# taraak/pita

Hardware: AMD Instinct MI355X
Metric: walker-steps/sec (batch x T) LJ13 @ 65k walkers/GPU (higher is better)
Workload: dtype f32

## Files before the change

### pita_amd/csrc/egnn_common.h

```cpp
#pragma once
#include <cstdlib>

#include "common.h"

namespace pita {

typedef float f32x16 __attribute__((ext_vector_type(16)));
typedef float f32x4 __attribute__((ext_vector_type(4)));

constexpr int EH = 32;
constexpr int PBS = 36;
constexpr int MAT_F = 1024;
enum { M_WA = 0, M_WB, M_W2, M_WC1, M_WN1A, M_WN1B, M_WN2,
       M_WAT, M_WBT, M_W2T, M_WC1T, M_WN1AT, M_WN1BT, M_WN2T, M_COUNT };
enum { V_WRE = 0 , V_B1 = 2, V_B2, V_WATT, V_BC1, V_WC2, V_BN1,
       V_BN2, V_WRF , V_WEF , V_COUNT };
constexpr int VEC_EMB_F = 96;
constexpr int VEC_LAYER_F = V_COUNT * EH + 4;


__device__ __forceinline__ void wave_lds_fence() {
  asm volatile("s_waitcnt lgkmcnt(0)" ::: "memory");
}

// ... 10 lines not shown
  const f32x4* p = reinterpret_cast<const f32x4*>(v);
  f32x4 a = p[0], b = p[1], c = p[2], d = p[3];
  f32x16 r;
  r[0] = a.x; r[1] = a.y; r[2] = a.z; r[3] = a.w;
  r[4] = b.x; r[5] = b.y; r[6] = b.z; r[7] = b.w;
  r[8] = c.x; r[9] = c.y; r[10] = c.z; r[11] = c.w;
  r[12] = d.x; r[13] = d.y; r[14] = d.z; r[15] = d.w;
  return r;
}

typedef short bf16x8 __attribute__((ext_vector_type(8)));
typedef unsigned int u32x4 __attribute__((ext_vector_type(4)));
constexpr int MAT_W = 1536;

template <int PREC>
struct WFrag;

template <>
struct WFrag<0> {
  float wf[16];
  __device__ __forceinline__ void load(const float* __restrict__ m32, const unsigned* __restrict__, int mat, int lane) {
    const f32x4* p = reinterpret_cast<const f32x4*>(m32 + (size_t)mat * MAT_F) + lane;
#pragma unroll
    for (int q = 0; q < 4; ++q) {
      f32x4 v = p[q * 64];
      wf[4 * q + 0] = v.x; wf[4 * q + 1] = v.y; wf[4 * q + 2] = v.z; wf[4 * q + 3] = v.w;
    }
  }
  __device__ __forceinline__ f32x16 mul(const f32x16& in, f32x16 acc) const {
#pragma unroll
    for (int r = 0; r < 16; ++r) acc = __builtin_amdgcn_mfma_f32_32x32x2f32(wf[r], in[r], acc, 0, 0, 0);
    return acc;
  }
};

__device__ __forceinline__ bf16x8 as_bf16x8(u32x4 v) { return __builtin_bit_cast(bf16x8, v); }

template <>
struct WFrag<1> {
  u32x4 w[3][2];
  __device__ __forceinline__ void load(const float* __restrict__, const unsigned* __restrict__ m16, int mat, int lane) {
    const u32x4* p = reinterpret_cast<const u32x4*>(m16 + (size_t)mat * MAT_W) + lane;
#pragma unroll
    for (int pc = 0; pc < 3; ++pc)
#pragma unroll
      for (int st = 0; st < 2; ++st) w[pc][st] = p[(pc * 2 + st) * 64];
  }
  static __device__ __forceinline__ void split(const f32x16& in, u32x4 (&x)[3][2]) {
#pragma unroll
    for (int st = 0; st < 2; ++st)
#pragma unroll
      for (int q = 0; q < 4; ++q) {
        typedef float f32x2_t __attribute__((ext_vector_type(2)));
        const unsigned a = __float_as_uint(in[8 * st + 2 * q]), b = __float_as_uint(in[8 * st + 2 * q + 1]);
        const unsigned a1 = a & 0xFFFF0000u, b1 = b & 0xFFFF0000u;
        const f32x2_t r1 = f32x2_t{__uint_as_float(a), __uint_as_float(b)} - f32x2_t{__uint_as_float(a1), __uint_as_float(b1)};
        const unsigned ar = __float_as_uint(r1.x), br = __float_as_uint(r1.y);
        const unsigned a2 = ar & 0xFFFF0000u, b2 = br & 0xFFFF0000u;
        const f32x2_t r2 = r1 - f32x2_t{__uint_as_float(a2), __uint_as_float(b2)};
        const unsigned a3 = __float_as_uint(r2.x), b3 = __float_as_uint(r2.y);
        x[0][st][q] = __builtin_amdgcn_perm(b1, a1, 0x07060302u);
        x[1][st][q] = __builtin_amdgcn_perm(b2, a2, 0x07060302u);
        x[2][st][q] = __builtin_amdgcn_perm(b3, a3, 0x07060302u);
      }
  }
  __device__ __forceinline__ f32x16 mul_split(const u32x4 (&x)[3][2], f32x16 acc) const {
#pragma unroll
    for (int st = 0; st < 2; ++st) {
      acc = __builtin_amdgcn_mfma_f32_32x32x16_bf16(as_bf16x8(w[2][st]), as_bf16x8(x[0][st]), acc, 0, 0, 0);
      acc = __builtin_amdgcn_mfma_f32_32x32x16_bf16(as_bf16x8(w[0][st]), as_bf16x8(x[2][st]), acc, 0, 0, 0);
      acc = __builtin_amdgcn_mfma_f32_32x32x16_bf16(as_bf16x8(w[1][st]), as_bf16x8(x[1][st]), acc, 0, 0, 0);
      acc = __builtin_amdgcn_mfma_f32_32x32x16_bf16(as_bf16x8(w[1][st]), as_bf16x8(x[0][st]), acc, 0, 0, 0);
      acc = __builtin_amdgcn_mfma_f32_32x32x16_bf16(as_bf16x8(w[0][st]), as_bf16x8(x[1][st]), acc, 0, 0, 0);
      acc = __builtin_amdgcn_mfma_f32_32x32x16_bf16(as_bf16x8(w[0][st]), as_bf16x8(x[0][st]), acc, 0, 0, 0);
    }
    return acc;
  }
  __device__ __forceinline__ f32x16 mul(const f32x16& in, f32x16 acc) const {
    u32x4 x[3][2];
    split(in, x);
    return mul_split(x, acc);
  }
};

constexpr float F16_SX = 1.0f, F16_SW = 16.0f;
constexpr bool F16_NODE_LAYERS = true;
constexpr float F16_UNSCALE = 1.0f / (F16_SX * F16_SW);
constexpr float DIV_ST = 32.0f;
constexpr float DIV_SV = 2048.0f;
constexpr int VEC_DIV_F = 4 * EH;
constexpr int MAT_WH = 1024;
typedef _Float16 f16x8 __attribute__((ext_vector_type(8)));
typedef _Float16 f16x2 __attribute__((ext_vector_type(2)));
__device__ __forceinline__ f16x8 as_f16x8(u32x4 v) { return __builtin_bit_cast(f16x8, v); }
__device__ __forceinline__ float f16_rem_lo(unsigned pk, float x) {
  float r;
  asm("v_fma_mix_f32 %0, %1, -1.0, %2 op_sel:[0,0,0] op_sel_hi:[1,0,0]" : "=v"(r) : "v"(pk), "v"(x));
  return r;
}
__device__ __forceinline__ float f16_rem_hi(unsigned pk, float x) {
  float r;
  asm("v_fma_mix_f32 %0, %1, -1.0, %2 op_sel:[1,0,0] op_sel_hi:[1,0,0]" : "=v"(r) : "v"(pk), "v"(x));
  return r;
}

template <>
struct WFrag<2> {
  u32x4 w[2][2];
  __device__ __forceinline__ void load(const float* __restrict__, const unsigned* __restrict__ m16, int mat, int lane) {
    const u32x4* p = reinterpret_cast<const u32x4*>(m16 + (size_t)mat * MAT_WH) + lane;
#pragma unroll
    for (int pc = 0; pc < 2; ++pc)
#pragma unroll
      for (int st = 0; st < 2; ++st) w[pc][st] = p[(pc * 2 + st) * 64];
  }
  static __device__ __forceinline__ void split(const f32x16& in, u32x4 (&x)[2][2]) {
    typedef float f32x2_t __attribute__((ext_vector_type(2)));
#pragma unroll
    for (int st = 0; st < 2; ++st)
#pragma unroll
      for (int q = 0; q < 4; ++q) {
        const float a = in[8 * st + 2 * q], b = in[8 * st + 2 * q + 1];
        const unsigned p1 = __builtin_bit_cast(unsigned, __builtin_convertvector(f32x2_t{a, b}, f16x2));
        const float ra = f16_rem_lo(p1, a), rb = f16_rem_hi(p1, b);
        x[0][st][q] = p1;
        x[1][st][q] = __builtin_bit_cast(unsigned, __builtin_convertvector(f32x2_t{ra, rb}, f16x2));
      }
  }
  __device__ __forceinline__ f32x16 mul_split(const u32x4 (&x)[2][2], f32x16 acc) const {
#pragma unroll
    for (int st = 0; st < 2; ++st) {
      acc = __builtin_amdgcn_mfma_f32_32x32x16_f16(as_f16x8(w[1][st]), as_f16x8(x[0][st]), acc, 0, 0, 0);
      acc = __builtin_amdgcn_mfma_f32_32x32x16_f16(as_f16x8(w[0][st]), as_f16x8(x[1][st]), acc, 0, 0, 0);
      acc = __builtin_amdgcn_mfma_f32_32x32x16_f16(as_f16x8(w[0][st]), as_f16x8(x[0][st]), acc, 0, 0, 0);
    }
    return acc;
  }
  __device__ __forceinline__ f32x16 mul(const f32x16& in, f32x16 acc) const {
    u32x4 x[2][2];
    split(in, x);
    return mul_split(x, acc);
  }
};

typedef float f32x2 __attribute__((ext_vector_type(2)));
constexpr float SILU_PRESCALE = -1.44269504088896341f;
__device__ __forceinline__ f32x2 silu2(f32x2 v) {
  f32x2 e;
  e.x = __builtin_amdgcn_exp2f(v.x);
  e.y = __builtin_amdgcn_exp2f(v.y);
  const f32x2 d = e + 1.0f;
  f32x2 r;
  r.x = __builtin_amdgcn_rcpf(d.x);
  r.y = __builtin_amdgcn_rcpf(d.y);
  return v * r;
}
__device__ __forceinline__ void silu16(f32x16& m) {
  f32x2 e[8];
#pragma unroll
  for (int q = 0; q < 8; ++q) {
    e[q].x = __builtin_amdgcn_exp2f(m[2 * q]);
    e[q].y = __builtin_amdgcn_exp2f(m[2 * q + 1]);
  }
#pragma unroll
  for (int q = 0; q < 8; ++q) e[q] = e[q] + 1.0f;
#pragma unroll
// ... 28 lines not shown
  const f32x2 c = {1.0f / F16_SX, 1.0f / F16_SX};
#pragma unroll
  for (int q0 = 0; q0 < 8; q0 += Q) {
    f32x2 v[Q], e[Q];
#pragma unroll
    for (int q = 0; q < Q; ++q) {
      v[q] = f32x2{m[2 * (q0 + q)], m[2 * (q0 + q) + 1]};
      if (UNSCALE) v[q] = v[q] * F16_UNSCALE;
    }
#pragma unroll
    for (int q = 0; q < Q; ++q) {
      e[q].x = __builtin_amdgcn_exp2f(v[q].x);
      e[q].y = __builtin_amdgcn_exp2f(v[q].y);
    }
#pragma unroll
    for (int q = 0; q < Q; ++q) e[q] = __builtin_elementwise_fma(e[q], c, c);
#pragma unroll
    for (int q = 0; q < Q; ++q) {
      e[q].x = __builtin_amdgcn_rcpf(e[q].x);
      e[q].y = __builtin_amdgcn_rcpf(e[q].y);
    }
#pragma unroll
    for (int q = 0; q < Q; ++q) {
      const f32x2 y = v[q] * e[q];
      m[2 * (q0 + q)] = y.x;
      m[2 * (q0 + q) + 1] = y.y;
    }
  }
}
__device__ __forceinline__ void silu16_out(f32x16& m) { silu16_staged<false>(m); }
__device__ __forceinline__ void silu16_acc(f32x16& m) { silu16_staged<true>(m); }

__device__ __forceinline__ float dot16(const f32x16& w, const f32x16& m) {
  f32x2 acc = {0.f, 0.f};
#pragma unroll
  for (int q = 0; q < 8; ++q)
    acc = __builtin_elementwise_fma(f32x2{w[2 * q], w[2 * q + 1]}, f32x2{m[2 * q], m[2 * q + 1]}, acc);
  return acc.x + acc.y;
}

__device__ __forceinline__ float xhalf_sum(float v) {
  const unsigned u = __float_as_uint(v);
  const auto r = __builtin_amdgcn_permlane32_swap(u, u, false, false);
  return __uint_as_float(r[0]) + __uint_as_float(r[1]);
}

__device__ __forceinline__ void frag_to_agpr(WFrag<2>& f) {
#pragma unroll
  for (int pc = 0; pc < 2; ++pc)
#pragma unroll
    for (int st = 0; st < 2; ++st) asm volatile("" : "+a"(f.w[pc][st]));
}
__device__ __forceinline__ void frag_to_agpr(WFrag<1>& f) {
#pragma unroll
  for (int pc = 0; pc < 3; ++pc)
#pragma unroll
    for (int st = 0; st < 2; ++st) asm volatile("" : "+a"(f.w[pc][st]));
}

__device__ __forceinline__ float tanh_select(float v) {
  const float a = fabsf(v);
  const float v2 = v * v;
  float p = 62.0f / 2835.0f;
  p = fmaf(p, v2, -17.0f / 315.0f);
  p = fmaf(p, v2, 2.0f / 15.0f);
  p = fmaf(p, v2, -1.0f / 3.0f);
  p = fmaf(p, v2, 1.0f);
  float small = v * p;
  const float e = __builtin_amdgcn_exp2f(2.88539008177792681f * a);
  float big = copysignf(1.0f - 2.0f * __builtin_amdgcn_rcpf(1.0f + e), v);
  asm volatile("" : "+v"(small), "+v"(big));
  return a < 0.25f ? small : big;
}

}

struct pita_egnn {
  pita_egnn_config cfg;
  unsigned* d_mats16 = nullptr;
  unsigned* d_mats16h = nullptr;
  float* d_mats = nullptr;
  float* d_vecs = nullptr;
  float* d_vecs_h = nullptr;
  float* d_vecs_div = nullptr;
  int* d_vjp_mark = nullptr;
  size_t vjp_mark_bytes = 0;
  const void* shape = nullptr;
  const void* shape_small = nullptr;
  int n_cu = 256;
  int device = -1;
  float* d_ws = nullptr;
  size_t ws_bytes = 0;
  float* d_divcache = nullptr;
  size_t divcache_bytes = 0;
  int* d_mark = nullptr;
  size_t mark_bytes = 0;
  int div_seq = 0;
  float* d_probe_q = nullptr;
  size_t probe_q_bytes = 0;
  void* d_bk = nullptr;
  size_t bk_bytes = 0;
};
```

### pita_amd/csrc/egnn_kernel.hip

```cpp
#include "egnn_common.h"

namespace pita {

struct EgnnParams {
  const unsigned* mats16;
  const unsigned* mats16h;
  const float* mats;
  const float* vecs;
  int n_layers, in_nf, attention, tanh_on, feature_layout;
  float coord_scale;
  int mode;
  long long B;
  const float* x_in;
  const float* t;
  const float* beta;
  float* out;
  float* x;
  const float* step_tab;
  int n_steps;
  const float* noise;
  unsigned long long seed, walker_offset;
  long long step0;
  int remove_mean;
  float* drift_out;
  double* stats_out;
  int repair;
  const float* x_backup;
  int* bad_from;
};

#ifndef PITA_EGNN_RECOMPUTE_COLS
#define PITA_EGNN_RECOMPUTE_COLS 1
#endif

template <int N, int DIM, int G, int WAVES>
struct EgnnCfg {
  static constexpr int NCOL = G * N;
  static constexpr int NT = (NCOL + 31) / 32;
  static constexpr int NCOLP = NT * 32;
  static constexpr int PB_F = NCOLP * PBS;
  static constexpr int POS_F = NCOLP * DIM;
  static constexpr int WAVE_F = PB_F + 4 * POS_F;
  static __host__ __device__ constexpr int vec_f(int L) { return ((VEC_EMB_F + L * VEC_LAYER_F) + 3) & ~3; }
  static __host__ __device__ constexpr size_t lds_bytes(int L) {
    return sizeof(float) * (size_t)(vec_f(L) + WAVES * WAVE_F);
  }
};

template <int N, int DIM, int G, int WAVES, int PREC, bool SAMPLER, int OCC = 2>
__global__ void __launch_bounds__(WAVES * 64, OCC) egnn_kernel(EgnnParams p) {
  const int mode = SAMPLER ? 3 : p.mode;
  using C = EgnnCfg<N, DIM, G, WAVES>;
  constexpr int NT = C::NT;
  extern __shared__ __attribute__((aligned(16))) float lds[];

  const int L = p.n_layers;
  const int vec_f = C::vec_f(L);
  for (int i = threadIdx.x; i < VEC_EMB_F + L * VEC_LAYER_F; i += WAVES * 64) lds[i] = p.vecs[i];
  __syncthreads();

  const int wave = threadIdx.x >> 6;
  const int lane = threadIdx.x & 63;
  const int cl = lane & 31;
  const int hh = lane >> 5;
  float* PB = lds + vec_f + wave * C::WAVE_F;
  float* posbuf0 = PB + C::PB_F;
  float* posbuf1 = posbuf0 + C::POS_F;
  float* pos0 = posbuf1 + C::POS_F;
  float* xbuf = pos0 + C::POS_F;
  const float* vemb = lds;

  const long long total_waves = (long long)gridDim.x * WAVES;
  const long long quota = (p.B + total_waves - 1) / total_waves;
  const long long wbeg = ((long long)blockIdx.x * WAVES + wave) * quota;
  const long long wend = (wbeg + quota < p.B) ? wbeg + quota : p.B;
  for (long long walker0 = wbeg; walker0 < wend; walker0 += G) {
    const int nwalk = (int)((wend - walker0) < G ? (wend - walker0) : G);
    const int ncol = nwalk * N;
    const int ntile = (ncol + 31) >> 5;
    int col[NT], nodei[NT];
    bool valid[NT];
    long long wid[NT];
    float xcur[NT][DIM];
#pragma unroll
    for (int T = 0; T < NT; ++T) {
      col[T] = T * 32 + cl;
      int w = col[T] / N;
      nodei[T] = col[T] - w * N;
      wid[T] = walker0 + w;
      valid[T] = (col[T] < ncol);
      if (!valid[T]) wid[T] = p.B - 1;
      const float* src = (mode == 3 ? p.x : p.x_in);
#pragma unroll
      for (int k = 0; k < DIM; ++k) xcur[T][k] = valid[T] ? src[(walker0 * N + col[T]) * DIM + k] : 0.0f;
    }
    int bad_from[NT];
#pragma unroll
    for (int T = 0; T < NT; ++T) bad_from[T] = 0x7fffffff;
    bool mine[NT];
#pragma unroll
    for (int T = 0; T < NT; ++T) mine[T] = valid[T];
    if (PREC != 2 && p.repair) {
      bool bad = false;
      float* flag = PB;
#pragma unroll
      for (int T = 0; T < NT; ++T) {
        bool b = false;
#pragma unroll
        for (int k = 0; k < DIM; ++k) {
          const float v = (mode == 3) ? xcur[T][k] : (valid[T] ? p.out[(walker0 * N + col[T]) * DIM + k] : 0.0f);
          b = b || !__builtin_isfinite(v);
        }
        if (hh == 0) flag[col[T]] = b ? 1.0f : 0.0f;
        bad = bad || b;
      }
      if (!__any(bad)) continue;
      wave_lds_fence();
#pragma unroll
      for (int T = 0; T < NT; ++T) {
        const int cb = (col[T] < ncol) ? col[T] - nodei[T] : 0;
        float any = 0.f;
        for (int q = 0; q < N; ++q) any += flag[cb + q];
        mine[T] = valid[T] && any != 0.f;
      }
      wave_lds_fence();
      if (mode == 3) {
#pragma unroll
        for (int T = 0; T < NT; ++T) {
#pragma unroll
          for (int k = 0; k < DIM; ++k)
            xcur[T][k] = valid[T] ? p.x_backup[(walker0 * N + col[T]) * DIM + k] : 0.0f;
          if (p.stats_out && p.bad_from && valid[T]) bad_from[T] = p.bad_from[walker0 * N + col[T]];
        }
      }
    }

// ... 38 lines not shown
          c_s[T] = u_cs; c_in[T] = u_cin; c_out[T] = u_cout;
          tfeat[T] = u_cn; hval[T] = u_h; bfeat[T] = u_b;
        }
        g2 = uni(PITA_ST_G2); gamma = uni(PITA_ST_GAMMA); dt = uni(PITA_ST_DT);
        noise_scale = uni(PITA_ST_NOISE_SCALE); sqrt_dt = uni(PITA_ST_SQRT_DT);
      } else {
#pragma unroll
        for (int T = 0; T < NT; ++T) {
          float tv = p.t[wid[T]];
          bfeat[T] = p.beta ? p.beta[wid[T]] : 0.0f;
          if (mode == 0) {
            c_s[T] = 0.f; c_in[T] = 1.f; c_out[T] = 1.f; tfeat[T] = tv; hval[T] = 1.f;
          } else {
            hval[T] = tv;
            c_s[T] = 1.0f / (1.0f + tv);
            c_in[T] = 1.0f / sqrtf(1.0f + tv);
            c_out[T] = sqrtf(tv) * c_in[T];
            tfeat[T] = 0.125f * logf(tv);
          }
        }
      }

      f32x16 hfeat[NT];
#pragma unroll
      for (int T = 0; T < NT; ++T) {
#pragma unroll
        for (int k = 0; k < DIM; ++k) {
          const float xc = xbuf[col[T] * DIM + k];
          const float ps = (mode == 0) ? xc : c_in[T] * xc;
          if (hh == 0) {
            pos0[col[T] * DIM + k] = ps;
            posbuf0[col[T] * DIM + k] = ps;
          }
        }
        float a0, a1;
        if (p.in_nf == 1) {
          a0 = tfeat[T]; a1 = 0.f;
        } else if (p.feature_layout == 0) {
          a0 = (2 * nodei[T] < N) ? tfeat[T] : bfeat[T];
          a1 = (2 * nodei[T] + 1 < N) ? tfeat[T] : bfeat[T];
        } else {
          a0 = tfeat[T]; a1 = bfeat[T];
        }
        f32x16 w0 = lds_vec16(vemb + hh * 16), w1 = lds_vec16(vemb + 32 + hh * 16), eb = lds_vec16(vemb + 64 + hh * 16);
#pragma unroll
        for (int r = 0; r < 16; ++r) hfeat[T][r] = fmaf(w0[r], a0, fmaf(w1[r], a1, eb[r]));
      }
      wave_lds_fence();

      float* poscur = posbuf0;
      float* posnext = posbuf1;
      for (int l = 0; l < L; ++l) {
        const float* mats = p.mats + (size_t)l * M_COUNT * MAT_F;
        const unsigned* mats16 = p.mats16 + (size_t)l * M_COUNT * MAT_W;
        const unsigned* mats16h = p.mats16h + (size_t)l * M_COUNT * MAT_WH;
        constexpr int NPREC = (PREC == 2 && !F16_NODE_LAYERS) ? 1 : PREC;
        constexpr bool NODE16 = (PREC == 2 && F16_NODE_LAYERS);
        const unsigned* matsn = NODE16 ? mats16h : mats16;
        const float* vl = lds + VEC_EMB_F + l * VEC_LAYER_F + hh * 16;
        const bool last = (l == L - 1);
        const float aggw = last ? 0.0f : (PREC == 2 ? 1.0f / F16_SX : 1.0f);
        {
          WFrag<NPREC> wb;
          wb.load(mats, matsn, M_WB, lane);
#pragma unroll
          for (int T = 0; T < NT; ++T) {
            if (T >= ntile) continue;
            f32x16 z = {0};
            f32x16 pb = wb.mul(hfeat[T], z);
            if (NODE16) pb *= F16_UNSCALE;
            f32x4* dst = reinterpret_cast<f32x4*>(PB + col[T] * PBS + hh * 16);
            dst[0] = f32x4{pb[0], pb[1], pb[2], pb[3]};
            dst[1] = f32x4{pb[4], pb[5], pb[6], pb[7]};
            dst[2] = f32x4{pb[8], pb[9], pb[10], pb[11]};
            dst[3] = f32x4{pb[12], pb[13], pb[14], pb[15]};
          }
        }
        wave_lds_fence();

        WFrag<PREC> w2f, wc1f;
        w2f.load(mats, PREC == 2 ? mats16h : mats16, M_W2, lane);
        wc1f.load(mats, PREC == 2 ? mats16h : mats16, M_WC1, lane);
        const float a_re = lds[VEC_EMB_F + l * VEC_LAYER_F + V_WRE * EH + lane];
        const float b_att = lds[VEC_EMB_F + l * VEC_LAYER_F + V_COUNT * EH];

#pragma unroll
        for (int T = 0; T < NT; ++T) {
          if (T >= ntile) continue;
          f32x16 Ai;
          {
            WFrag<NPREC> wa;
            wa.load(mats, matsn, M_WA, lane);
            Ai = wa.mul(hfeat[T], lds_vec16(vl + V_B1 * EH));
            if (NODE16) Ai *= F16_UNSCALE;
          }
          f32x16 agg = {0};
          float xacc[DIM], pown[DIM], p0own[DIM];
#pragma unroll
          for (int k = 0; k < DIM; ++k) {
            xacc[k] = 0.f;
            pown[k] = poscur[col[T] * DIM + k];
            p0own[k] = pos0[col[T] * DIM + k];
          }
          const int cbase = col[T] - nodei[T];

          for (int dd = 1; dd < N; ++dd) {
            asm volatile("" ::: "memory");
            int j = nodei[T] + dd;
            j = (j >= N) ? j - N : j;
            const int cj = (col[T] < ncol) ? cbase + j : col[T];
            float df[DIM], radial = 0.f, ea = 0.f;
#pragma unroll
            for (int k = 0; k < DIM; ++k) {
              df[k] = pown[k] - poscur[cj * DIM + k];
              radial = fmaf(df[k], df[k], radial);
              const float e0 = p0own[k] - pos0[cj * DIM + k];
              ea = fmaf(e0, e0, ea);
            }
            f32x16 m = Ai + lds_vec16(PB + cj * PBS + hh * 16);
            m = __builtin_amdgcn_mfma_f32_32x32x2f32(a_re, hh ? ea : radial, m, 0, 0, 0);
            __builtin_amdgcn_s_setprio(0);
            if (PREC == 2) silu16_out(m); else silu16(m);
            __builtin_amdgcn_s_setprio(1);
            m = w2f.mul(m, lds_vec16(vl + V_B2 * EH));
            __builtin_amdgcn_s_setprio(0);
            if (PREC == 2) silu16_acc(m); else silu16(m);
            __builtin_amdgcn_s_setprio(1);
            if (p.attention) {
              const float att = fast_sigmoid(xhalf_sum(dot16(lds_vec16(vl + V_WATT * EH), m)) + b_att);
              m *= att;
            }
#pragma unroll
            for (int r = 0; r < 16; ++r) agg[r] = fmaf(m[r], aggw, agg[r]);
            f32x16 c1 = wc1f.mul(m, lds_vec16(vl + V_BC1 * EH));
            __builtin_amdgcn_s_setprio(0);
            if (PREC == 2) silu16_acc(c1); else silu16(c1);
            __builtin_amdgcn_s_setprio(1);
            float cs = xhalf_sum(dot16(lds_vec16(vl + V_WC2 * EH), c1));
            if (p.tanh_on) cs = accurate_tanh(cs) * p.coord_scale;
            const float inrm = __builtin_amdgcn_rcpf(__builtin_amdgcn_sqrtf(radial + 1e-8f) + 1.0f);
#pragma unroll
            for (int k = 0; k < DIM; ++k) xacc[k] = fmaf(df[k] * inrm, cs, xacc[k]);
          }
#pragma unroll
          for (int k = 0; k < DIM; ++k) {
            if (hh == 0) posnext[col[T] * DIM + k] = pown[k] + xacc[k];
          }
          if (!last) {
            WFrag<NPREC> wn;
            wn.load(mats, matsn, M_WN1A, lane);
            f32x16 n1 = wn.mul(hfeat[T], lds_vec16(vl + V_BN1 * EH));
            wn.load(mats, matsn, M_WN1B, lane);
            n1 = wn.mul(agg, n1);
            if (NODE16) silu16_acc(n1); else if (PREC == 2) silu16_out(n1); else silu16(n1);
            WFrag<PREC> wo;
            wo.load(mats, PREC == 2 ? mats16h : mats16, M_WN2, lane);
            f32x16 o = wo.mul(n1, lds_vec16(vl + V_BN2 * EH));
            if (PREC == 2) o *= F16_UNSCALE;
            hfeat[T] += o;
          }
        }
        wave_lds_fence();
        float* tmp = poscur; poscur = posnext; posnext = tmp;
      }

      float* scr = PB;
      float F[NT][DIM];
#pragma unroll
      for (int T = 0; T < NT; ++T)
#pragma unroll
        for (int k = 0; k < DIM; ++k) {
          F[T][k] = poscur[col[T] * DIM + k] - pos0[col[T] * DIM + k];
          if (hh == 0) scr[col[T] * DIM + k] = F[T][k];
        }
      wave_lds_fence();
#pragma unroll
      for (int T = 0; T < NT; ++T) {
        const int cb = (col[T] < ncol) ? col[T] - nodei[T] : 0;
#pragma unroll
        for (int k = 0; k < DIM; ++k) {
          float s = 0.f;
          for (int q = 0; q < N; ++q) s += scr[(cb + q) * DIM + k];
          F[T][k] -= s / (float)N;
        }
      }
      wave_lds_fence();

      if (mode != 3) {
#pragma unroll
        for (int T = 0; T < NT; ++T)
#pragma unroll
          for (int k = 0; k < DIM; ++k) {
            float o = F[T][k];
            if (mode >= 1) {
              const float xc = xbuf[col[T] * DIM + k];
              o = c_s[T] * xc + c_out[T] * F[T][k];
              if (mode == 2) o = (o - xc) / hval[T];
            }
            if (mine[T] && hh == 0) p.out[(walker0 * N + col[T]) * DIM + k] = o;
          }
      } else {
        float xn[NT][DIM];
        float st_d = 0.f, st_d2 = 0.f, st_n = 0.f, st_n2 = 0.f;
#pragma unroll
        for (int T = 0; T < NT; ++T) {
          float xi[4] = {0.f, 0.f, 0.f, 0.f};
          if (p.noise) {
#pragma unroll
            for (int k = 0; k < DIM; ++k)
              xi[k] = valid[T] ? p.noise[((size_t)step * p.B * N + (size_t)(walker0 * N + col[T])) * DIM + k] : 0.f;
          } else {
            philox_normal4(p.seed, p.walker_offset + (unsigned long long)wid[T], p.step0 + step, (uint32_t)nodei[T], xi);
          }
          bool take_col = true;
          if (p.stats_out && valid[T] && hh == 0) {
            if (PREC == 2) {
#pragma unroll
              for (int k = 0; k < DIM; ++k) {
                const float xc = xbuf[col[T] * DIM + k];
                const float Dth = c_s[T] * xc + c_out[T] * F[T][k];
                take_col = take_col && __builtin_isfinite(gamma * (((Dth - xc) / hval[T]) * g2));
              }
              take_col = take_col && bad_from[T] == 0x7fffffff;
              if (!take_col && bad_from[T] == 0x7fffffff) bad_from[T] = step;
            } else if (p.repair) {
              take_col = step >= bad_from[T];
            }
          }
#pragma unroll
          for (int k = 0; k < DIM; ++k) {
            const float xc = xbuf[col[T] * DIM + k];
            const float Dth = c_s[T] * xc + c_out[T] * F[T][k];
            const float sc = (Dth - xc) / hval[T];
            const float drift = gamma * (sc * g2);
            if (p.drift_out && step == nsteps - 1 && mine[T] && hh == 0)
              p.drift_out[(walker0 * N + col[T]) * DIM + k] = drift;
            const float dif = noise_scale * xi[k];
            if (p.stats_out && valid[T] && hh == 0) {
              const bool take = take_col;
              if (take) {
                st_d += drift; st_d2 = fmaf(drift, drift, st_d2);
                st_n += dif; st_n2 = fmaf(dif, dif, st_n2);
              }
            }
            xn[T][k] = xc + (drift * dt + (dif * sqrt_dt));
            if (hh == 0) scr[col[T] * DIM + k] = xn[T][k];
          }
        }
        if (p.stats_out) {
          double m4[4] = {(double)st_d, (double)st_d2, (double)st_n, (double)st_n2};
#pragma unroll
          for (int q = 0; q < 4; ++q) {
            for (int o = 32; o > 0; o >>= 1) m4[q] += __shfl_xor(m4[q], o, 64);
            if (lane == 0) atomicAdd(p.stats_out + (size_t)step * 4 + q, m4[q]);
          }
        }
        if (p.remove_mean) {
          wave_lds_fence();
#pragma unroll
          for (int T = 0; T < NT; ++T) {
            const int cb = (col[T] < ncol) ? col[T] - nodei[T] : 0;
#pragma unroll
            for (int k = 0; k < DIM; ++k) {
              float s = 0.f;
              for (int q = 0; q < N; ++q) s += scr[(cb + q) * DIM + k];
              xn[T][k] -= s / (float)N;
            }
          }
          wave_lds_fence();
        }
#pragma unroll
        for (int T = 0; T < NT; ++T)
#pragma unroll
          for (int k = 0; k < DIM; ++k)
            if (hh == 0) xbuf[col[T] * DIM + k] = xn[T][k];
        wave_lds_fence();
      }
    }

    if (mode == 3) {
#pragma unroll
      for (int T = 0; T < NT; ++T) {
#pragma unroll
        for (int k = 0; k < DIM; ++k)
          if (mine[T] && hh == 0) p.x[(walker0 * N + col[T]) * DIM + k] = xbuf[col[T] * DIM + k];
        if (PREC == 2 && p.stats_out && p.bad_from && valid[T] && hh == 0) p.bad_from[walker0 * N + col[T]] = bad_from[T];
      }
    }
    wave_lds_fence();
  }
}


struct EgnnShape {
  int n, dim, G, waves, occ;
  void (*kernel[3][2])(EgnnParams);
  size_t (*lds_bytes)(int);
};

template <int N, int DIM, int G, int WAVES>
static size_t lds_bytes_of(int L) { return EgnnCfg<N, DIM, G, WAVES>::lds_bytes(L); }

#define PITA_EGNN_SHAPE(N, DIM, G, WAVES, OCC) \
  EgnnShape { N, DIM, G, WAVES, OCC, \
              {{egnn_kernel<N, DIM, G, WAVES, 0, false, OCC>, egnn_kernel<N, DIM, G, WAVES, 0, true, OCC>}, \
               {egnn_kernel<N, DIM, G, WAVES, 1, false, OCC>, egnn_kernel<N, DIM, G, WAVES, 1, true, OCC>}, \
               {egnn_kernel<N, DIM, G, WAVES, 2, false, OCC>, egnn_kernel<N, DIM, G, WAVES, 2, true, OCC>}}, \
              lds_bytes_of<N, DIM, G, WAVES> }

static const EgnnShape kShapes[] = {
    PITA_EGNN_SHAPE(4, 2, 8, 4, 2),
    PITA_EGNN_SHAPE(13, 3, 7, 4, 2),
    PITA_EGNN_SHAPE(22, 3, 4, 4, 2),
    PITA_EGNN_SHAPE(55, 3, 1, 4, 2),
};
static const EgnnShape kShapesSmall[] = {
    PITA_EGNN_SHAPE(13, 3, 2, 4, 2),
    PITA_EGNN_SHAPE(22, 3, 2, 4, 2),
};

}


using namespace pita;

extern "C" int64_t pita_egnn_num_weights(const pita_egnn_config* c) {
  if (!c) return PITA_EINVAL;
  const int64_t H = c->hidden_nf;
  int64_t per_layer = (H * (2 * H + 2) + H) + (H * H + H) + (H * 2 * H + H) + (H * H + H) + (H * H + H) + H;
  if (c->attention) per_layer += H + 1;
  return (H * c->in_node_nf + H) + (c->in_node_nf * H + c->in_node_nf) + c->n_layers * per_layer;
}

static inline int kfeat(int r, int hh) { return (r & 3) + 8 * (r >> 2) + 4 * hh; }

extern "C" int pita_egnn_create(pita_egnn_t** out, const pita_egnn_config* cfg, const float* w, int64_t n_weights) {
  PITA_REQUIRE(out && cfg && w, "pita_egnn_create: null argument");
  if (cfg->hidden_nf != EH)
    return fail(PITA_EUNSUPPORTED, "pita_egnn_create: hidden_nf=%d (the HIP kernel implements 32)", cfg->hidden_nf);
  PITA_REQUIRE(cfg->in_node_nf == 1 || cfg->in_node_nf == 2, "in_node_nf must be 1 or 2");
  PITA_REQUIRE(cfg->precision >= 0 && cfg->precision <= 2,
               "precision must be 0 (f32 MFMA), 1 (bf16 three-piece split) or 2 (f16 two-piece split)");
  PITA_REQUIRE(cfg->n_layers >= 1 && cfg->n_layers <= 16, "n_layers out of range");
  PITA_REQUIRE(n_weights == pita_egnn_num_weights(cfg), "pita_egnn_create: got %lld weights, expected %lld",
               (long long)n_weights, (long long)pita_egnn_num_weights(cfg));
  const EgnnShape* shape = nullptr;
  const EgnnShape* shape_small = nullptr;
  for (const auto& s : kShapes)
    if (s.n == cfg->n_particles && s.dim == cfg->n_dim) shape = &s;
  for (const auto& s : kShapesSmall)
    if (s.n == cfg->n_particles && s.dim == cfg->n_dim) shape_small = &s;
  if (!shape)
    return fail(PITA_EUNSUPPORTED, "pita_egnn_create: no kernel for %d particles in %d dimensions", cfg->n_particles,
                cfg->n_dim);
  const int H = EH, L = cfg->n_layers, nf = cfg->in_node_nf;
  const size_t n_mats = (size_t)L * M_COUNT * MAT_F, n_vecs = VEC_EMB_F + (size_t)L * VEC_LAYER_F;
  float* h_mats = new float[n_mats];
  float* h_vecs = new float[n_vecs]();
  const size_t n_mats16 = (size_t)L * M_COUNT * MAT_W;
  unsigned* h_mats16 = new unsigned[n_mats16];
  const size_t n_mats16h = (size_t)L * M_COUNT * MAT_WH;
  unsigned* h_mats16h = new unsigned[n_mats16h]();
  float* h_vecs_h = new float[n_vecs]();
  float* h_vecs_div = new float[(size_t)L * VEC_DIV_F]();
  const float* q = w;
  const float* emb_w = q; q += H * nf;
  const float* emb_b = q; q += H;
  q += nf * H + nf;
  for (int hh = 0; hh < 2; ++hh)
    for (int r = 0; r < 16; ++r) {
      const int f = kfeat(r, hh);
      h_vecs[hh * 16 + r] = emb_w[f * nf + 0];
      h_vecs[32 + hh * 16 + r] = (nf == 2) ? emb_w[f * nf + 1] : 0.f;
      h_vecs[64 + hh * 16 + r] = emb_b[f];
    }
  const float kS = SILU_PRESCALE, kSi = 1.0f / SILU_PRESCALE;
  auto pack_mat = [&](float* dst, const float* M, int ld, int col0, float sc) {
    for (int qd = 0; qd < 4; ++qd)
      for (int lane = 0; lane < 64; ++lane)
        for (int s = 0; s < 4; ++s)
          dst[(qd * 64 + lane) * 4 + s] = sc * M[(lane & 31) * ld + col0 + kfeat(4 * qd + s, lane >> 5)];
  };
  auto trunc16 = [](float v) { unsigned u; memcpy(&u, &v, 4); u &= 0xFFFF0000u; float o; memcpy(&o, &u, 4); return o; };
  auto hi16 = [](float v) { unsigned u; memcpy(&u, &v, 4); return u >> 16; };
  auto pack_mat16 = [&](unsigned* dst, const float* M, int ld, int col0, float sc) {
    for (int lane = 0; lane < 64; ++lane)
      for (int st = 0; st < 2; ++st)
        for (int qd = 0; qd < 4; ++qd) {
          unsigned pcs[2][3];
          for (int e = 0; e < 2; ++e) {
            const float w = sc * M[(lane & 31) * ld + col0 + kfeat(8 * st + 2 * qd + e, lane >> 5)];
            const float w1 = trunc16(w), r1 = w - w1, w2 = trunc16(r1), r2 = r1 - w2;
            pcs[e][0] = hi16(w1); pcs[e][1] = hi16(w2); pcs[e][2] = hi16(r2);
          }
          for (int pc = 0; pc < 3; ++pc)
            dst[(((size_t)pc * 2 + st) * 64 + lane) * 4 + qd] = pcs[0][pc] | (pcs[1][pc] << 16);
        }
  };
  auto f16_bits = [](float v) { _Float16 h = (_Float16)v; unsigned short u; memcpy(&u, &h, 2); return (unsigned)u; };
  auto pack_mat16h = [&](unsigned* dst, const float* M, int ld, int col0, float sc) {
    for (int lane = 0; lane < 64; ++lane)
      for (int st = 0; st < 2; ++st)
        for (int qd = 0; qd < 4; ++qd) {
          unsigned pcs[2][2];
          for (int e = 0; e < 2; ++e) {
            const float w = F16_SW * (sc * M[(lane & 31) * ld + col0 + kfeat(8 * st + 2 * qd + e, lane >> 5)]);
            const _Float16 w1 = (_Float16)w;
            pcs[e][0] = f16_bits((float)w1);
            pcs[e][1] = f16_bits(w - (float)w1);
          }
          for (int pc = 0; pc < 2; ++pc)
            dst[(((size_t)pc * 2 + st) * 64 + lane) * 4 + qd] = pcs[0][pc] | (pcs[1][pc] << 16);
        }
  };
  auto pack_vec = [&](float* dst, const float* v, int stride, float sc) {
    for (int hh = 0; hh < 2; ++hh)
      for (int r = 0; r < 16; ++r) dst[hh * 16 + r] = sc * v[kfeat(r, hh) * stride];
  };
  for (int l = 0; l < L; ++l) {
    float* mats = h_mats + (size_t)l * M_COUNT * MAT_F;
    float* vecs = h_vecs + VEC_EMB_F + (size_t)l * VEC_LAYER_F;
    const float* e0w = q; q += H * (2 * H + 2);
    const float* e0b = q; q += H;
    const float* e2w = q; q += H * H;
    const float* e2b = q; q += H;
    const float* n0w = q; q += H * 2 * H;
    const float* n0b = q; q += H;
    const float* n2w = q; q += H * H;
    const float* n2b = q; q += H;
    const float* c0w = q; q += H * H;
    const float* c0b = q; q += H;
    const float* c2w = q; q += H;
    const float* aw = nullptr; const float* ab = nullptr;
    if (cfg->attention) { aw = q; q += H; ab = q; q += 1; }
    unsigned* m16 = h_mats16 + (size_t)l * M_COUNT * MAT_W;
    pack_mat16(m16 + M_WA * MAT_W, e0w, 2 * H + 2, 0, kS);
    pack_mat16(m16 + M_WB * MAT_W, e0w, 2 * H + 2, H, kS);
    pack_mat16(m16 + M_W2 * MAT_W, e2w, H, 0, 1.0f);
    pack_mat16(m16 + M_WC1 * MAT_W, c0w, H, 0, 1.0f);
    pack_mat16(m16 + M_WN1A * MAT_W, n0w, 2 * H, 0, kS);
    pack_mat16(m16 + M_WN1B * MAT_W, n0w, 2 * H, H, 1.0f);
    pack_mat16(m16 + M_WN2 * MAT_W, n2w, H, 0, kSi);
    unsigned* m16h = h_mats16h + (size_t)l * M_COUNT * MAT_WH;
    pack_mat16h(m16h + M_WA * MAT_WH, e0w, 2 * H + 2, 0, kS);
    pack_mat16h(m16h + M_WB * MAT_WH, e0w, 2 * H + 2, H, kS);
    pack_mat16h(m16h + M_W2 * MAT_WH, e2w, H, 0, 1.0f);
    pack_mat16h(m16h + M_WC1 * MAT_WH, c0w, H, 0, 1.0f);
    pack_mat16h(m16h + M_WN1A * MAT_WH, n0w, 2 * H, 0, kS);
    pack_mat16h(m16h + M_WN1B * MAT_WH, n0w, 2 * H, H, 1.0f);
    pack_mat16h(m16h + M_WN2 * MAT_WH, n2w, H, 0, kSi);
    pack_mat(mats + M_WA * MAT_F, e0w, 2 * H + 2, 0, kS);
    pack_mat(mats + M_WB * MAT_F, e0w, 2 * H + 2, H, kS);
    pack_mat(mats + M_W2 * MAT_F, e2w, H, 0, 1.0f);
    pack_mat(mats + M_WC1 * MAT_F, c0w, H, 0, 1.0f);
    pack_mat(mats + M_WN1A * MAT_F, n0w, 2 * H, 0, kS);
    pack_mat(mats + M_WN1B * MAT_F, n0w, 2 * H, H, 1.0f);
    pack_mat(mats + M_WN2 * MAT_F, n2w, H, 0, kSi);
    {
      float T[EH * EH];
      auto pack_t = [&](int slot, const float* M, int ld, int col0) {
        for (int k = 0; k < H; ++k)
          for (int o = 0; o < H; ++o) T[k * H + o] = M[o * ld + col0 + k];
        pack_mat16(m16 + slot * MAT_W, T, H, 0, 1.0f);
        pack_mat(mats + slot * MAT_F, T, H, 0, 1.0f);
      };
      auto pack_th = [&](int slot, const float* M, int ld, int col0) {
        for (int k = 0; k < H; ++k)
          for (int o = 0; o < H; ++o) T[k * H + o] = M[o * ld + col0 + k];
        pack_mat16h(m16h + slot * MAT_WH, T, H, 0, 1.0f);
      };
      pack_th(M_W2T, e2w, H, 0);
      pack_th(M_WC1T, c0w, H, 0);
      pack_t(M_WAT, e0w, 2 * H + 2, 0);
      pack_t(M_WBT, e0w, 2 * H + 2, H);
      pack_t(M_W2T, e2w, H, 0);
      pack_t(M_WC1T, c0w, H, 0);
      pack_t(M_WN1AT, n0w, 2 * H, 0);
      pack_t(M_WN1BT, n0w, 2 * H, H);
      pack_t(M_WN2T, n2w, H, 0);
    }
    for (int o = 0; o < H; ++o) {
      vecs[V_WRE * EH + o] = kS * e0w[o * (2 * H + 2) + 2 * H];
      vecs[V_WRE * EH + H + o] = kS * e0w[o * (2 * H + 2) + 2 * H + 1];
    }
    pack_vec(vecs + V_B1 * EH, e0b, 1, kS);
    pack_vec(vecs + V_B2 * EH, e2b, 1, kS);
    if (aw) pack_vec(vecs + V_WATT * EH, aw, 1, kSi);
    pack_vec(vecs + V_BC1 * EH, c0b, 1, kS);
    pack_vec(vecs + V_WC2 * EH, c2w, 1, kSi);
    pack_vec(vecs + V_BN1 * EH, n0b, 1, kS);
    pack_vec(vecs + V_BN2 * EH, n2b, 1, 1.0f);
    pack_vec(vecs + V_WRF * EH, e0w + 2 * H, 2 * H + 2, 1.0f);
    pack_vec(vecs + V_WEF * EH, e0w + 2 * H + 1, 2 * H + 2, 1.0f);
    {
      float* vd = h_vecs_div + (size_t)l * VEC_DIV_F;
      pack_vec(vd + EH, e0w + 2 * H, 2 * H + 2, kS);
      pack_vec(vd + 2 * EH, e0w + 2 * H + 1, 2 * H + 2, kS);
      for (int o = 0; o < H; ++o) vd[o] = DIV_ST * (vd[EH + o] + vd[2 * EH + o]);
      pack_vec(vd + 3 * EH, c2w, 1, DIV_SV * kSi);
    }
    vecs[V_COUNT * EH] = ab ? ab[0] : 0.f;
    {
      float* vh = h_vecs_h + VEC_EMB_F + (size_t)l * VEC_LAYER_F;
      memcpy(vh, vecs, sizeof(float) * VEC_LAYER_F);
      const float up = F16_SX * F16_SW, dn = 1.0f / F16_SX;
      for (int o = 0; o < H; ++o) {
        vh[V_B2 * EH + o] *= up; vh[V_BC1 * EH + o] *= up; vh[V_BN2 * EH + o] *= up;
        if (F16_NODE_LAYERS) { vh[V_B1 * EH + o] *= up; vh[V_BN1 * EH + o] *= up; }
        vh[V_WATT * EH + o] *= dn; vh[V_WC2 * EH + o] *= dn;
      }
    }
  }
  memcpy(h_vecs_h, h_vecs, sizeof(float) * VEC_EMB_F);
  pita_egnn* net = new pita_egnn();
  net->cfg = *cfg;
  net->shape = shape;
  net->shape_small = shape_small;
  hipError_t e1 = hipMalloc(&net->d_mats, n_mats * sizeof(float));
  hipError_t e2 = hipMalloc(&net->d_vecs, n_vecs * sizeof(float));
  hipError_t e0 = hipMalloc(&net->d_mats16, n_mats16 * sizeof(unsigned));
  if (e0 == hipSuccess) e0 = hipMalloc(&net->d_mats16h, n_mats16h * sizeof(unsigned));
  if (e0 == hipSuccess) e0 = hipMalloc(&net->d_vecs_h, n_vecs * sizeof(float));
  if (e0 == hipSuccess) e0 = hipMalloc(&net->d_vecs_div, (size_t)L * VEC_DIV_F * sizeof(float));
  if (e0 == hipSuccess)
    e0 = hipMemcpy(net->d_vecs_div, h_vecs_div, (size_t)L * VEC_DIV_F * sizeof(float), hipMemcpyHostToDevice);
  if (e0 == hipSuccess) e0 = hipMemcpy(net->d_mats16h, h_mats16h, n_mats16h * sizeof(unsigned), hipMemcpyHostToDevice);
  if (e0 == hipSuccess) e0 = hipMemcpy(net->d_vecs_h, h_vecs_h, n_vecs * sizeof(float), hipMemcpyHostToDevice);
  if (e1 == hipSuccess && e2 == hipSuccess && e0 == hipSuccess) {
    e1 = hipMemcpy(net->d_mats, h_mats, n_mats * sizeof(float), hipMemcpyHostToDevice);
    e2 = hipMemcpy(net->d_vecs, h_vecs, n_vecs * sizeof(float), hipMemcpyHostToDevice);
    e0 = hipMemcpy(net->d_mats16, h_mats16, n_mats16 * sizeof(unsigned), hipMemcpyHostToDevice);
  }
  if (e0 != hipSuccess && e1 == hipSuccess) e1 = e0;
  delete[] h_mats;
  delete[] h_vecs;
  delete[] h_mats16;
  delete[] h_mats16h;
  delete[] h_vecs_h;
  delete[] h_vecs_div;
  if (e1 != hipSuccess || e2 != hipSuccess) {
    (void)hipFree(net->d_mats);
    (void)hipFree(net->d_vecs);
    (void)hipFree(net->d_mats16);
    (void)hipFree(net->d_mats16h);
    (void)hipFree(net->d_vecs_h);
    (void)hipFree(net->d_vecs_div);
    delete net;
    return fail(PITA_EHIP, "pita_egnn_create: device upload failed: %s",
                hipGetErrorString(e1 != hipSuccess ? e1 : e2));
  }
  int dev = 0;
  hipDeviceProp_t prop;
  if (hipGetDevice(&dev) == hipSuccess) {
    net->device = dev;
    if (hipGetDeviceProperties(&prop, dev) == hipSuccess) net->n_cu = prop.multiProcessorCount;
  }
  size_t lds = shape->lds_bytes(L);
  hipError_t e3 = hipSuccess;
  for (int a = 0; a < 3 && e3 == hipSuccess; ++a)
    for (int b = 0; b < 2 && e3 == hipSuccess; ++b) {
      e3 = ensure_dynamic_lds(reinterpret_cast<const void*>(shape->kernel[a][b]), lds);
      if (e3 == hipSuccess && shape_small)
        e3 = ensure_dynamic_lds(reinterpret_cast<const void*>(shape_small->kernel[a][b]), shape_small->lds_bytes(L));
    }
  if (e3 != hipSuccess) {
    pita_egnn_destroy(net);
    return fail(PITA_EHIP, "pita_egnn_create: cannot reserve %zu B of LDS: %s", lds, hipGetErrorString(e3));
  }
  *out = net;
  return PITA_OK;
}

extern "C" int pita_egnn_destroy(pita_egnn_t* net) {
  if (!net) return PITA_OK;
  PitaDeviceGuard guard(net->device);
  (void)hipFree(net->d_mats);
  (void)hipFree(net->d_vecs);
  (void)hipFree(net->d_mats16);
  (void)hipFree(net->d_vjp_mark);
  (void)hipFree(net->d_mats16h);
  (void)hipFree(net->d_vecs_h);
  (void)hipFree(net->d_vecs_div);
  (void)hipFree(net->d_ws);
  (void)hipFree(net->d_bk);
  (void)hipFree(net->d_mark);
  (void)hipFree(net->d_divcache);
  (void)hipFree(net->d_probe_q);
  delete net;
  return PITA_OK;
}

static const EgnnShape* shape_for(const pita_egnn_t* net, long long B) {
  const EgnnShape* s = static_cast<const EgnnShape*>(net->shape);
  const EgnnShape* t = static_cast<const EgnnShape*>(net->shape_small);
  if (!t) return s;
  const long long two_per_simd = (long long)net->n_cu * 8;
  const long long waves_s = (B + s->G - 1) / s->G;
  return waves_s < two_per_simd ? t : s;
}

struct EgnnMapping {
  const EgnnShape* s;
  size_t lds;
  long long want, cap;
  long long grid() const { return want < cap ? want : cap; }
};
static EgnnMapping egnn_mapping(const pita_egnn_t* net, long long B) {
  const EgnnShape* s = shape_for(net, B);
  const size_t lds = s->lds_bytes(net->cfg.n_layers);
  int blocks_per_cu = (int)((160 * 1024) / lds);
  blocks_per_cu = blocks_per_cu < 1 ? 1 : (blocks_per_cu > s->occ ? s->occ : blocks_per_cu);
  const long long ngroups = (B + s->G - 1) / s->G;
  return {s, lds, (ngroups + s->waves - 1) / s->waves, (long long)net->n_cu * blocks_per_cu};
}

static int egnn_launch(pita_egnn_t* net, EgnnParams& p, void* stream) {
  PitaDeviceGuard guard(net->device);
  const int prec = net->cfg.precision;
  p.mats = net->d_mats;
  p.mats16 = net->d_mats16;
  p.mats16h = net->d_mats16h;
  p.vecs = prec == 2 ? net->d_vecs_h : net->d_vecs;
  p.n_layers = net->cfg.n_layers;
  p.in_nf = net->cfg.in_node_nf;
  p.attention = net->cfg.attention;
  p.tanh_on = net->cfg.tanh;
  p.feature_layout = net->cfg.feature_layout;
  p.coord_scale = net->cfg.coords_range / (float)net->cfg.n_layers;
  if (p.B == 0) return PITA_OK;
  const EgnnMapping m = egnn_mapping(net, p.B);
  const EgnnShape* s = m.s;
  const size_t lds = m.lds;
  const int smp = p.mode == 3 ? 1 : 0;
  const unsigned grid = (unsigned)(smp ? m.grid() : m.want);
  if (prec == 2 && smp) {
    PITA_HIP_CHECK(grow_scratch(net->d_bk, net->bk_bytes,
                                sizeof(float) * (size_t)p.B * s->n * s->dim + sizeof(int) * (size_t)p.B * s->n,
                                (hipStream_t)stream));
    float* xb = static_cast<float*>(net->d_bk);
    PITA_HIP_CHECK(hipMemcpyAsync(xb, p.x, sizeof(float) * (size_t)p.B * s->n * s->dim, hipMemcpyDeviceToDevice,
                                  (hipStream_t)stream));
    p.x_backup = xb;
    p.bad_from = reinterpret_cast<int*>(xb + (size_t)p.B * s->n * s->dim);
  }
  hipLaunchKernelGGL(s->kernel[prec][smp], dim3(grid), dim3(s->waves * 64), lds, (hipStream_t)stream, p);
  PITA_LAUNCH_CHECK();
  if (prec == 2) {
    p.repair = 1;
    p.vecs = net->d_vecs;
    hipLaunchKernelGGL(s->kernel[1][smp], dim3(grid), dim3(s->waves * 64), lds, (hipStream_t)stream, p);
    PITA_LAUNCH_CHECK();
  }
  return PITA_OK;
}

extern "C" int pita_egnn_sampler_work(const pita_egnn_t* net, int64_t B, double* mfma16_per_walker_step,
                                      double* mfma32_per_walker_step) {
  PITA_REQUIRE(net && B > 0 && mfma16_per_walker_step && mfma32_per_walker_step, "pita_egnn_sampler_work: bad argument");
  const EgnnMapping m = egnn_mapping(net, B);
  const int L = net->cfg.n_layers, N = m.s->n, G = m.s->G;
  const long long total_waves = m.grid() * m.s->waves;
  const long long quota = (B + total_waves - 1) / total_waves;
  double tiles = 0.0;
  for (long long wbeg = 0; wbeg < B; wbeg += quota) {
    const long long wend = wbeg + quota < B ? wbeg + quota : B;
    for (long long w0 = wbeg; w0 < wend; w0 += G) {
      const long long nw = (wend - w0) < G ? (wend - w0) : G;
      tiles += (double)((nw * N + 31) / 32);
    }
  }
  const double node_dense = tiles * (L * 2.0 + (L - 1) * 2.0);
  const double edge_dense = tiles * (L * 2.0 * (N - 1) + (L - 1) * 1.0);
  const double kstep = tiles * L * (N - 1);
  if (net->cfg.precision == 0) {
    *mfma16_per_walker_step = 0.0;
    *mfma32_per_walker_step = (16.0 * (node_dense + edge_dense) + kstep) / (double)B;
  } else {
    const double f16d = net->cfg.precision == 2 ? 6.0 : 12.0;
    *mfma16_per_walker_step = ((F16_NODE_LAYERS ? f16d : 12.0) * node_dense + f16d * edge_dense) / (double)B;
    *mfma32_per_walker_step = kstep / (double)B;
  }
  return PITA_OK;
}

extern "C" int pita_egnn_sampler_mapping(const pita_egnn_t* net, int64_t B, int* walkers_per_group, int64_t* waves,
                                         int64_t* wave_slots) {
  PITA_REQUIRE(net && B > 0 && walkers_per_group && waves && wave_slots, "pita_egnn_sampler_mapping: bad argument");
  const EgnnMapping m = egnn_mapping(net, B);
  *walkers_per_group = m.s->G;
  *waves = m.grid() * m.s->waves;
  *wave_slots = m.cap * m.s->waves;
  return PITA_OK;
}

extern "C" int pita_egnn_forward(pita_egnn_t* net, const float* t, const float* x, const float* beta, float* out,
                                 int64_t B, void* stream) {
  PITA_REQUIRE(net && t && x && out && B >= 0, "pita_egnn_forward: null argument");
  PITA_REQUIRE(beta || net->cfg.in_node_nf == 1, "pita_egnn_forward: beta required for in_node_nf=2");
  EgnnParams p{};
  p.mode = 0; p.B = B; p.x_in = x; p.t = t; p.beta = beta; p.out = out;
  return egnn_launch(net, p, stream);
}

extern "C" int pita_egnn_edm(pita_egnn_t* net, int what, const float* h, const float* x, const float* beta, float* out,
                             int64_t B, void* stream) {
  PITA_REQUIRE(net && h && x && out && B >= 0, "pita_egnn_edm: null argument");
  PITA_REQUIRE(what == 1 || what == 2, "pita_egnn_edm: what must be 1 (denoiser) or 2 (score)");
  PITA_REQUIRE(beta || net->cfg.in_node_nf == 1, "pita_egnn_edm: beta required for in_node_nf=2");
  EgnnParams p{};
  p.mode = what; p.B = B; p.x_in = x; p.t = h; p.beta = beta; p.out = out;
  return egnn_launch(net, p, stream);
}

extern "C" int pita_egnn_sampler_run(pita_egnn_t* net, float* x, int64_t B, const float* step_tab, int n_steps,
                                     const float* noise, uint64_t seed, uint64_t walker_offset, int64_t step0,
                                     int remove_mean, float* drift_out, double* stats_out, void* stream) {
  PITA_REQUIRE(net && x && step_tab && B >= 0 && n_steps >= 0, "pita_egnn_sampler_run: bad argument");
  if (n_steps == 0) return PITA_OK;
  EgnnParams p{};
  p.mode = 3; p.B = B; p.x = x; p.step_tab = step_tab; p.n_steps = n_steps; p.noise = noise;
  p.seed = seed; p.walker_offset = walker_offset; p.step0 = step0; p.remove_mean = remove_mean;
  p.drift_out = drift_out; p.stats_out = stats_out;
  return egnn_launch(net, p, stream);
}
```

Before: 62.38 million.

## Use split-bf16 MFMA for radial k-step and defer attention gating past Wc1

For N=13 with reduced precision, the per-edge radial/edge-attribute rank-2 update is moved from the fp32 32x32x2 MFMA to a single bf16 32x32x16 MFMA. Both operands are split into three bf16 pieces (host-precomputed weight triples, device-side split of the scalar), which keeps near-fp32 accuracy. In the PREC==2 path, the attention scale is applied after the Wc1 matmul rather than to m beforehand, and its unscale and bias are folded into one FMA. This takes a multiply off the critical chain and uses a separate bias vector buffer. The aim is to cut per-edge latency on the slow fp32 MFMA, at the cost of extra VALU split work.

```diff
diff --git a/pita_amd/csrc/egnn_common.h b/pita_amd/csrc/egnn_common.h
--- a/pita_amd/csrc/egnn_common.h
+++ b/pita_amd/csrc/egnn_common.h
@@ -116,6 +116,19 @@
     return mul_split(x, acc);
   }
 };
+
+__device__ __forceinline__ bf16x8 kstep_split(float s) {
+  const unsigned s1 = __float_as_uint(s) & 0xFFFF0000u;
+  const float q1 = s - __uint_as_float(s1);
+  const unsigned s2 = __float_as_uint(q1) & 0xFFFF0000u;
+  const float q2 = q1 - __uint_as_float(s2);
+  const unsigned s3 = __float_as_uint(q2);
+  const unsigned s12 = __builtin_amdgcn_perm(s2, s1, 0x07060302u);
+  return as_bf16x8(u32x4{s12, __builtin_amdgcn_perm(s3, s1, 0x07060302u), s12, __builtin_amdgcn_perm(s2, s3, 0x07060302u)});
+}
+__device__ __forceinline__ f32x16 kstep_mul(u32x4 a, float s, f32x16 acc) {
+  return __builtin_amdgcn_mfma_f32_32x32x16_bf16(as_bf16x8(a), kstep_split(s), acc, 0, 0, 0);
+}
 
 constexpr float F16_SX = 1.0f, F16_SW = 16.0f;
 constexpr bool F16_NODE_LAYERS = true;
@@ -310,6 +323,8 @@
   float* d_mats = nullptr;
   float* d_vecs = nullptr;
   float* d_vecs_h = nullptr;
+  float* d_vecs_s = nullptr;
+  unsigned* d_kstep16 = nullptr;
   float* d_vecs_div = nullptr;
   int* d_vjp_mark = nullptr;
   size_t vjp_mark_bytes = 0;
diff --git a/pita_amd/csrc/egnn_kernel.hip b/pita_amd/csrc/egnn_kernel.hip
--- a/pita_amd/csrc/egnn_kernel.hip
+++ b/pita_amd/csrc/egnn_kernel.hip
@@ -7,6 +7,7 @@
   const unsigned* mats16h;
   const float* mats;
   const float* vecs;
+  const unsigned* kstep16;
   int n_layers, in_nf, attention, tanh_on, feature_layout;
   float coord_scale;
   int mode;
@@ -41,6 +42,7 @@
   static constexpr int PB_F = NCOLP * PBS;
   static constexpr int POS_F = NCOLP * DIM;
   static constexpr int WAVE_F = PB_F + 4 * POS_F;
+  static constexpr bool KSTEP_GATE = (N == 13);
   static __host__ __device__ constexpr int vec_f(int L) { return ((VEC_EMB_F + L * VEC_LAYER_F) + 3) & ~3; }
   static __host__ __device__ constexpr size_t lds_bytes(int L) {
     return sizeof(float) * (size_t)(vec_f(L) + WAVES * WAVE_F);
@@ -52,6 +54,8 @@
   const int mode = SAMPLER ? 3 : p.mode;
   using C = EgnnCfg<N, DIM, G, WAVES>;
   constexpr int NT = C::NT;
+  constexpr bool KSTEP16 = C::KSTEP_GATE && PREC != 0;
+  constexpr bool GATE_POST = C::KSTEP_GATE && PREC == 2;
   extern __shared__ __attribute__((aligned(16))) float lds[];
 
   const int L = p.n_layers;
@@ -256,6 +260,8 @@
         w2f.load(mats, PREC == 2 ? mats16h : mats16, M_W2, lane);
         wc1f.load(mats, PREC == 2 ? mats16h : mats16, M_WC1, lane);
         const float a_re = lds[VEC_EMB_F + l * VEC_LAYER_F + V_WRE * EH + lane];
+        u32x4 a_re16 = {0, 0, 0, 0};
+        if (KSTEP16) a_re16 = reinterpret_cast<const u32x4*>(p.kstep16)[l * 64 + lane];
         const float b_att = lds[VEC_EMB_F + l * VEC_LAYER_F + V_COUNT * EH];
 
 #pragma unroll
@@ -292,7 +298,8 @@
               ea = fmaf(e0, e0, ea);
             }
             f32x16 m = Ai + lds_vec16(PB + cj * PBS + hh * 16);
-            m = __builtin_amdgcn_mfma_f32_32x32x2f32(a_re, hh ? ea : radial, m, 0, 0, 0);
+            if (KSTEP16) m = kstep_mul(a_re16, hh ? ea : radial, m);
+            else m = __builtin_amdgcn_mfma_f32_32x32x2f32(a_re, hh ? ea : radial, m, 0, 0, 0);
             __builtin_amdgcn_s_setprio(0);
             if (PREC == 2) silu16_out(m); else silu16(m);
             __builtin_amdgcn_s_setprio(1);
@@ -300,15 +307,29 @@
             __builtin_amdgcn_s_setprio(0);
             if (PREC == 2) silu16_acc(m); else silu16(m);
             __builtin_amdgcn_s_setprio(1);
-            if (p.attention) {
-              const float att = fast_sigmoid(xhalf_sum(dot16(lds_vec16(vl + V_WATT * EH), m)) + b_att);
-              m *= att;
+            f32x16 c1;
+            if (GATE_POST) {
+              f32x16 z = {0};
+              c1 = wc1f.mul(m, z);
+              float att = 1.0f;
+              if (p.attention) att = fast_sigmoid(xhalf_sum(dot16(lds_vec16(vl + V_WATT * EH), m)) + b_att);
+              const float ga = att * aggw, gc = att * F16_UNSCALE;
+#pragma unroll
+              for (int r = 0; r < 16; ++r) agg[r] = fmaf(m[r], ga, agg[r]);
+              const f32x16 bc1 = lds_vec16(vl + V_BC1 * EH);
+#pragma unroll
+              for (int r = 0; r < 16; ++r) c1[r] = fmaf(c1[r], gc, bc1[r]);
+            } else {
+              if (p.attention) {
+                const float att = fast_sigmoid(xhalf_sum(dot16(lds_vec16(vl + V_WATT * EH), m)) + b_att);
+                m *= att;
+              }
+#pragma unroll
+              for (int r = 0; r < 16; ++r) agg[r] = fmaf(m[r], aggw, agg[r]);
+              c1 = wc1f.mul(m, lds_vec16(vl + V_BC1 * EH));
             }
-#pragma unroll
-            for (int r = 0; r < 16; ++r) agg[r] = fmaf(m[r], aggw, agg[r]);
-            f32x16 c1 = wc1f.mul(m, lds_vec16(vl + V_BC1 * EH));
             __builtin_amdgcn_s_setprio(0);
-            if (PREC == 2) silu16_acc(c1); else silu16(c1);
+            if (GATE_POST) silu16_out(c1); else if (PREC == 2) silu16_acc(c1); else silu16(c1);
             __builtin_amdgcn_s_setprio(1);
             float cs = xhalf_sum(dot16(lds_vec16(vl + V_WC2 * EH), c1));
             if (p.tanh_on) cs = accurate_tanh(cs) * p.coord_scale;
@@ -468,6 +489,7 @@
 
 struct EgnnShape {
   int n, dim, G, waves, occ;
+  bool kstep_gate;
   void (*kernel[3][2])(EgnnParams);
   size_t (*lds_bytes)(int);
 };
@@ -476,7 +498,7 @@
 static size_t lds_bytes_of(int L) { return EgnnCfg<N, DIM, G, WAVES>::lds_bytes(L); }
 
 #define PITA_EGNN_SHAPE(N, DIM, G, WAVES, OCC) \
-  EgnnShape { N, DIM, G, WAVES, OCC, \
+  EgnnShape { N, DIM, G, WAVES, OCC, EgnnCfg<N, DIM, G, WAVES>::KSTEP_GATE, \
               {{egnn_kernel<N, DIM, G, WAVES, 0, false, OCC>, egnn_kernel<N, DIM, G, WAVES, 0, true, OCC>}, \
                {egnn_kernel<N, DIM, G, WAVES, 1, false, OCC>, egnn_kernel<N, DIM, G, WAVES, 1, true, OCC>}, \
                {egnn_kernel<N, DIM, G, WAVES, 2, false, OCC>, egnn_kernel<N, DIM, G, WAVES, 2, true, OCC>}}, \
@@ -537,6 +559,7 @@
   unsigned* h_mats16h = new unsigned[n_mats16h]();
   float* h_vecs_h = new float[n_vecs]();
   float* h_vecs_div = new float[(size_t)L * VEC_DIV_F]();
+  unsigned* h_kstep16 = new unsigned[(size_t)L * 64 * 4];
   const float* q = w;
   const float* emb_w = q; q += H * nf;
   const float* emb_b = q; q += H;
@@ -657,6 +680,13 @@
       vecs[V_WRE * EH + o] = kS * e0w[o * (2 * H + 2) + 2 * H];
       vecs[V_WRE * EH + H + o] = kS * e0w[o * (2 * H + 2) + 2 * H + 1];
     }
+    for (int lane = 0; lane < 64; ++lane) {
+      const float w = vecs[V_WRE * EH + lane];
+      const float w1 = trunc16(w), r1 = w - w1, w2 = trunc16(r1), r2 = r1 - w2;
+      const unsigned p1 = hi16(w1), p2 = hi16(w2), p3 = hi16(r2);
+      unsigned* a = h_kstep16 + ((size_t)l * 64 + lane) * 4;
+      a[0] = p1 | (p1 << 16); a[1] = p2 | (p1 << 16); a[2] = p3 | (p2 << 16); a[3] = p2 | (p3 << 16);
+    }
     pack_vec(vecs + V_B1 * EH, e0b, 1, kS);
     pack_vec(vecs + V_B2 * EH, e2b, 1, kS);
     if (aw) pack_vec(vecs + V_WATT * EH, aw, 1, kSi);
@@ -700,6 +730,16 @@
     e0 = hipMemcpy(net->d_vecs_div, h_vecs_div, (size_t)L * VEC_DIV_F * sizeof(float), hipMemcpyHostToDevice);
   if (e0 == hipSuccess) e0 = hipMemcpy(net->d_mats16h, h_mats16h, n_mats16h * sizeof(unsigned), hipMemcpyHostToDevice);
   if (e0 == hipSuccess) e0 = hipMemcpy(net->d_vecs_h, h_vecs_h, n_vecs * sizeof(float), hipMemcpyHostToDevice);
+  if (e0 == hipSuccess) e0 = hipMalloc(&net->d_kstep16, (size_t)L * 64 * 4 * sizeof(unsigned));
+  if (e0 == hipSuccess)
+    e0 = hipMemcpy(net->d_kstep16, h_kstep16, (size_t)L * 64 * 4 * sizeof(unsigned), hipMemcpyHostToDevice);
+  for (int l = 0; l < L; ++l)
+    for (int o = 0; o < H; ++o) {
+      const size_t i = VEC_EMB_F + (size_t)l * VEC_LAYER_F + V_BC1 * EH + o;
+      h_vecs_h[i] = h_vecs[i];
+    }
+  if (e0 == hipSuccess) e0 = hipMalloc(&net->d_vecs_s, n_vecs * sizeof(float));
+  if (e0 == hipSuccess) e0 = hipMemcpy(net->d_vecs_s, h_vecs_h, n_vecs * sizeof(float), hipMemcpyHostToDevice);
   if (e1 == hipSuccess && e2 == hipSuccess && e0 == hipSuccess) {
     e1 = hipMemcpy(net->d_mats, h_mats, n_mats * sizeof(float), hipMemcpyHostToDevice);
     e2 = hipMemcpy(net->d_vecs, h_vecs, n_vecs * sizeof(float), hipMemcpyHostToDevice);
@@ -712,12 +752,15 @@
   delete[] h_mats16h;
   delete[] h_vecs_h;
   delete[] h_vecs_div;
+  delete[] h_kstep16;
   if (e1 != hipSuccess || e2 != hipSuccess) {
     (void)hipFree(net->d_mats);
     (void)hipFree(net->d_vecs);
     (void)hipFree(net->d_mats16);
     (void)hipFree(net->d_mats16h);
     (void)hipFree(net->d_vecs_h);
+    (void)hipFree(net->d_vecs_s);
+    (void)hipFree(net->d_kstep16);
     (void)hipFree(net->d_vecs_div);
     delete net;
     return fail(PITA_EHIP, "pita_egnn_create: device upload failed: %s",
@@ -754,6 +797,8 @@
   (void)hipFree(net->d_vjp_mark);
   (void)hipFree(net->d_mats16h);
   (void)hipFree(net->d_vecs_h);
+  (void)hipFree(net->d_vecs_s);
+  (void)hipFree(net->d_kstep16);
   (void)hipFree(net->d_vecs_div);
   (void)hipFree(net->d_ws);
   (void)hipFree(net->d_bk);
@@ -794,7 +839,7 @@
   p.mats = net->d_mats;
   p.mats16 = net->d_mats16;
   p.mats16h = net->d_mats16h;
-  p.vecs = prec == 2 ? net->d_vecs_h : net->d_vecs;
+  p.kstep16 = net->d_kstep16;
   p.n_layers = net->cfg.n_layers;
   p.in_nf = net->cfg.in_node_nf;
   p.attention = net->cfg.attention;
@@ -804,6 +849,7 @@
   if (p.B == 0) return PITA_OK;
   const EgnnMapping m = egnn_mapping(net, p.B);
   const EgnnShape* s = m.s;
+  p.vecs = prec == 2 ? (s->kstep_gate ? net->d_vecs_s : net->d_vecs_h) : net->d_vecs;
   const size_t lds = m.lds;
   const int smp = p.mode == 3 ? 1 : 0;
   const unsigned grid = (unsigned)(smp ? m.grid() : m.want);
@@ -851,8 +897,9 @@
     *mfma32_per_walker_step = (16.0 * (node_dense + edge_dense) + kstep) / (double)B;
   } else {
     const double f16d = net->cfg.precision == 2 ? 6.0 : 12.0;
-    *mfma16_per_walker_step = ((F16_NODE_LAYERS ? f16d : 12.0) * node_dense + f16d * edge_dense) / (double)B;
-    *mfma32_per_walker_step = kstep / (double)B;
+    const double k16 = m.s->kstep_gate ? kstep : 0.0;
+    *mfma16_per_walker_step = ((F16_NODE_LAYERS ? f16d : 12.0) * node_dense + f16d * edge_dense + k16) / (double)B;
+    *mfma32_per_walker_step = (kstep - k16) / (double)B;
   }
   return PITA_OK;
 }
```

After: 62.91 million (median of 6 runs). No clear change (+0.9%).
